# jacobwulffwold/GAN_SR_wind_field

Hardware: AMD Instinct MI355X
Metric: GAN train-steps/sec (G+D fwd+bwd) (higher is better)
Workload: dtype bf16; 1 GPU; C3' full G+D adversarial step: LR 32x32x128 -> HR 128x128x128 (x4), batch 1/GPU, G 16 RRDB nf128 (34.77M), D bf32; preset=C3p, global_batch=1, parallelism=dp1, ranks=1

## Files before the change

### gan_sr_wind_field_amd/_lib.py

```python
from __future__ import annotations

import ctypes as C
import os
from typing import Optional

_HERE = os.path.dirname(os.path.abspath(__file__))
LIB_PATH = os.environ.get("WSR_LIB_PATH") or os.path.join(_HERE, "csrc", "libwindsr_hip.so")

WSR_F32, WSR_BF16 = 0, 1
WSR_EUNSUPPORTED = -2

EXPORTS = [
    "wsr_abi_version", "wsr_error_string", "wsr_reload_env", "wsr_ragan_loss", "wsr_bn_train_stats", "wsr_conv3d_fwd", "wsr_conv3d_dgrad", "wsr_conv3d_wgrad", "wsr_conv3d_wgrad_tri", "wsr_conv3d_wgrad_nparts", "wsr_conv3d_wgrad_parts", "wsr_conv3d_wgrad_parts_x2", "wsr_conv_split_ok", "wsr_unpack_wgrad_reduce_multi", "wsr_conv3d_fwd_tile", "wsr_conv3d_dgrad_tile",
    "wsr_frag_filter_elems", "wsr_pack_filter_frag", "wsr_pack_filter_frag_multi",
    "wsr_pack_filter", "wsr_unpack_wgrad", "wsr_unpack_wgrad_multi", "wsr_lrelu_bwd_inplace", "wsr_chan_axpby", "wsr_chan_sum", "wsr_chan_sum_rows", "wsr_chan_sum_partials", "wsr_upsample2_bwd", "wsr_subpixel_fold", "wsr_subpixel_unfold", "wsr_strided_parity_filters", "wsr_strided_parity_unfold",
    "wsr_planar_to_ndhwc", "wsr_ndhwc_to_planar", "wsr_zfold", "wsr_zunfold", "wsr_wind_gradient", "wsr_wind_gradient_bwd", "wsr_plane_sum", "wsr_linear_rows", "wsr_physics_loss_workspace_floats", "wsr_physics_loss_stats", "wsr_physics_loss_bwd", "wsr_bn_stats", "wsr_bn_mean", "wsr_bn_shard_stats", "wsr_bn_combine_shards", "wsr_bn_finalize", "wsr_bn_apply_lrelu", "wsr_bn_bwd_reduce",
    "wsr_bn_bwd_apply", "wsr_adam_step", "wsr_adam_multi", "wsr_gather_batch",
]


class ConvDesc(C.Structure):

    _fields_ = [(n, C.c_int32) for n in (
        "dtype", "B", "Xi", "Yi", "Zi", "Xo", "Yo", "Zo", "Cin", "in_ctot", "in_off", "Cout", "out_ctot",
        "out_off", "KX", "KY", "KZ", "sx", "sy", "sz", "px", "py", "pz", "upsample_xy", "lat", "lat_ox", "lat_oy",
        "lat_phases", "lat_mz", "lat_oz")]


class Epilogue(C.Structure):

    _fields_ = [
        ("bias", C.c_void_p), ("chan_scale", C.c_void_p), ("res", C.c_void_p),
# ... 78 lines not shown
        "wsr_physics_loss_bwd": [vp, vp, vp, vp, vp, vp, vp, vp, i32, i32, i32, i32, vp],
        "wsr_zunfold": [vp, vp, i32, i32, i32, i32, i64, i32, i32, i32, i32, i32, vp],
        "wsr_bn_stats": [vp, i32, i64, vp, vp, vp, i32, vp],
        "wsr_bn_mean": [vp, vp, f32, vp, i32, vp],
        "wsr_bn_shard_stats": [vp, i32, vp, i32, f32, vp, i32, i32, vp],
        "wsr_bn_combine_shards": [vp, i32, f32, vp, i32, vp, i32, i32, i32, vp],
        "wsr_bn_finalize": [vp, vp, f32, vp, f32, f32, vp, vp, vp, vp, i32, vp],
        "wsr_bn_apply_lrelu": [vp, vp, vp, vp, vp, vp, i32, i64, i32, f32, i32, vp],
        "wsr_bn_bwd_reduce": [vp, vp, vp, vp, vp, i32, i64, i32, f32, vp, vp, i32, vp],
        "wsr_bn_bwd_apply": [vp, vp, vp, vp, vp, vp, vp, f32, vp, f32, i32, i64, i32, vp],
        "wsr_adam_step": [vp, vp, vp, vp, i64, f32, f32, f32, f32, f32, i32, vp],
        "wsr_adam_multi": [vp, i32, C.c_double, C.c_double, C.c_double, C.c_double, C.c_double, i32, vp],
        "wsr_ragan_loss": [vp, vp, vp, vp, vp, vp, i32, vp, vp],
        "wsr_bn_train_stats": [vp, i32, i64, i32, f32, f32, vp, vp, vp, vp, i32, vp],
        "wsr_gather_batch": [vp, i64, vp, i32, i32, i32, i32, i32, i32, i32, vp, vp, vp, vp],
    }
    for name, argtypes in sig.items():
        fn = getattr(L, name)
        fn.argtypes = argtypes
        fn.restype = C.c_int
    L.wsr_frag_filter_elems.argtypes = [i32, i32, i32, i32]
    L.wsr_frag_filter_elems.restype = C.c_int64
    L.wsr_physics_loss_workspace_floats.argtypes = []
    L.wsr_physics_loss_workspace_floats.restype = C.c_int64
    if L.wsr_abi_version() != 9:
        raise RuntimeError("libwindsr_hip.so ABI version mismatch")
    _lib = L
    return L


# ... 5 lines not shown
```

### gan_sr_wind_field_amd/csrc/conv_wgrad.hip

```cpp
#include "common.h"

namespace {

typedef __attribute__((ext_vector_type(4))) short s16x4_t;
typedef s16x4_t __attribute__((address_space(3))) * lds_s16x4_ptr;

struct WgradArgs {
  const char* x;
  const char* dy;
  float* dw;
  int B, Xi, Yi, Zi, Xo, Yo, Zo;
  int Cin, in_ctot, in_off;
  int Cout, out_ctot, out_off;
  int KX, KY, KZ, sx, sy, sz, px, py, pz, ups;
  int M;
  int mchunk;
  int ntiles, ctiles;
  long part_stride;
  int mchunks;
};

template <class T> struct WgCfg;
template <> struct WgCfg<BF16> { static constexpr int KB = 128; };
template <> struct WgCfg<F32> { static constexpr int KB = 64; };
// ... 194 lines not shown

template <class T>
int dispatch_wgrad(WgradArgs& a, hipStream_t st, int* plan, int n_parts) {
  if (a.Cout % 48 == 0 && a.Cin % 48 == 0 && a.Cin % 64 != 0) return launch_wgrad<T, 3, 3>(a, st, plan, n_parts);
  if (a.Cout <= 16)
    return a.Cin <= 16 ? launch_wgrad<T, 1, 1>(a, st, plan, n_parts) : launch_wgrad<T, 1, 4>(a, st, plan, n_parts);
  if (a.Cin <= 16) return launch_wgrad<T, 2, 1>(a, st, plan, n_parts);
  if (a.Cin <= 32) return launch_wgrad<T, 2, 2>(a, st, plan, n_parts);
  return launch_wgrad<T, 2, 4>(a, st, plan, n_parts);
}

}

int wsr_wgrad_tile_bf16(const wsr_conv_t* c, const void* x, const void* dy, float* dw, int tri_base, int tri_step,
                        long part_stride, int n_parts, int* plan, void* stream, const void* x2, int x2_ctot,
                        int x2_c0);

int wsr_wgrad_tile_f32(const wsr_conv_t* c, const void* x, const void* dy, float* dw, long part_stride, int n_parts,
                       int* plan, void* stream, const void* x2, int x2_ctot, int x2_c0);

static int wgrad_any(const wsr_conv_t* c, const void* x, const void* dy, float* dw, int tri_base, int tri_step,
                     long part_stride, int n_parts, int* plan, void* stream, const void* x2 = nullptr, int x2_ctot = 0,
                     int x2_c0 = 0) {
  {
    const int rc = wsr_wgrad_tile_bf16(c, x, dy, dw, tri_base, tri_step, part_stride, n_parts, plan, stream, x2, x2_ctot,
                                       x2_c0);
    if (rc != WSR_EUNSUPPORTED || tri_step > 0) return rc;
  }
  if (c->lat) return WSR_EUNSUPPORTED;
  if (c->dtype == WSR_F32 && tri_step == 0) {
    const int rc = wsr_wgrad_tile_f32(c, x, dy, dw, part_stride, n_parts, plan, stream, x2, x2_ctot, x2_c0);
    if (rc != WSR_EUNSUPPORTED) return rc;
  }
  if (x2) return WSR_EUNSUPPORTED;
  const int epp = c->dtype == WSR_BF16 ? 8 : 4;
  if (c->Cin % epp || c->in_ctot % epp || c->in_off % epp) return WSR_EUNSUPPORTED;
  if (c->out_ctot % epp || c->out_off % epp) return WSR_EUNSUPPORTED;
  if ((long)c->B * c->Xo * c->Yo * c->Zo > 0x7fffffffL) return WSR_EUNSUPPORTED;
  WgradArgs a{};
  a.x = (const char*)x;
  a.dy = (const char*)dy;
// ... 39 lines not shown

extern "C" int wsr_conv3d_wgrad_parts(const wsr_conv_t* c, const void* x, const void* dy, float* parts,
                                      int64_t part_stride, int32_t n_parts, int32_t tri_base, int32_t tri_step,
                                      void* stream) {
  if (!conv_geom_ok(c) || !x || !dy || !parts || tri_base < 0 || tri_step < 0 || n_parts <= 0) return WSR_EINVAL;
  if (part_stride < (int64_t)c->Cout * c->KX * c->KY * c->KZ * c->Cin) return WSR_EINVAL;
  return wgrad_any(c, x, dy, parts, tri_base, tri_step, (long)part_stride, n_parts, nullptr, stream);
}

extern "C" int wsr_conv3d_wgrad_parts_x2(const wsr_conv_t* c, const void* x, const void* x2, int32_t x2_ctot, int32_t x2_c0,
                                         const void* dy, float* parts, int64_t part_stride, int32_t n_parts, void* stream) {
  if (!conv_geom_ok_split(c, x2_c0) || !x || !x2 || !dy || !parts || n_parts <= 0 || x2_ctot <= 0) return WSR_EINVAL;
  if (part_stride < (int64_t)c->Cout * c->KX * c->KY * c->KZ * c->Cin) return WSR_EINVAL;
  return wgrad_any(c, x, dy, parts, 0, 0, (long)part_stride, n_parts, nullptr, stream, x2, x2_ctot, x2_c0);
}
```

### gan_sr_wind_field_amd/csrc/conv_wgrad_tile.hip

```cpp
#include <cstdlib>

#include "common.h"

namespace {

typedef __attribute__((ext_vector_type(4))) short s16x4_t;
typedef s16x4_t __attribute__((address_space(3))) * lds_s16x4_ptr;

struct WgtArgs {
  const unsigned short* x;
  const unsigned short* x2;
  int x2_ctot, x2_c0;
  const unsigned short* dy;
  float* dw;
  const void* zero16;
  int B, Xi, Yi, Zi, Xo, Yo, Zo;
  int Cin, in_ctot, in_off;
  int Cout, out_ctot, out_off;
  int KX, KY, KZ, px, py, pz, ups;
  int TX, TY, TZ;
  int n_chunks, c_chunks, S;
  int tiles_x, tiles_y, tiles_z, ntiles;
  int nbuf;
  int xp_bytes;
// ... 449 lines not shown
  const int taps = a.KX * a.KY * a.KZ;
  if (taps * CT > WAVES * SPW) return WSR_EUNSUPPORTED;
  if (a.x2 && a.x2_c0 % (16 * CT)) return WSR_EUNSUPPORTED;
  {
    static void* zp = nullptr;
    if (!zp) {
      hipError_t e = hipGetSymbolAddress(&zp, HIP_SYMBOL(g_wg_zero16));
      if (e != hipSuccess) return (int)e;
    }
    a.zero16 = zp;
  }
  int tz = a.Zo <= 16 ? a.Zo : ((a.Zo % 16 == 0 || a.Zo > 64) ? 16 : 8);
  if (a.KZ == 1 && a.KX * a.KY > 1 && tz > 4 && a.Zo % 4 == 0 && !WSR_ENV_SET("WSR_CT_NOFLAT")) tz = 4;
  static const int cand[][2] = {{8, 8}, {4, 8}, {4, 4}, {2, 4}, {2, 2}, {1, 2}, {1, 1}};
  int best = -1, best_nbuf = 0;
  const int nbuf_want = taps == 1 ? WSR_ENV_INT("WSR_WG_NBUF", 2) : ((SPW == 4 && CT == 1) ? WSR_ENV_INT("WSR_WG_NBUF_THIN", 2) : 2);
  const int mmax = taps == 1 && nbuf_want > 2 ? WSR_ENV_INT("WSR_WG_MMAX", 64) : 1 << 30;
  for (int nbuf = nbuf_want; nbuf >= 2 && best < 0; --nbuf) {
    for (int ci = 0; ci < 7; ++ci) {
      const int tx = cand[ci][0], ty = cand[ci][1];
      const int M = tx * ty * tz;
      if ((M & 31) || M > mmax) continue;
      if (a.ups && ((tx | ty) & 1)) continue;
      const int L = (tx + a.KX - 1) * (ty + a.KY - 1) * (tz + a.KZ - 1);
      const int xs = CT * round_up(L * 32, 1024), ys = round_up(M * wgt_rby(TN), 1024);
      if (xs / 1024 > wgt_xk(SPW, TN) * WAVES || ys / 1024 > wgt_yk(SPW, TN) * WAVES || L > 65535) continue;
      if (round_up(M * 2, 1024) + nbuf * (xs + ys) > 160 * 1024) continue;
      best = ci;
      best_nbuf = nbuf;
      break;
    }
  }
  if (best < 0) return WSR_EUNSUPPORTED;
  a.TX = cand[best][0]; a.TY = cand[best][1]; a.TZ = tz;
  a.nbuf = best_nbuf;
  const int M = a.TX * a.TY * a.TZ;
  const int L = (a.TX + a.KX - 1) * (a.TY + a.KY - 1) * (a.TZ + a.KZ - 1);
// ... 46 lines not shown
    hipError_t e = hipFuncSetAttribute(reinterpret_cast<const void*>(kern), hipFuncAttributeMaxDynamicSharedMemorySize,
                                       160 * 1024);
    if (e != hipSuccess) return (int)e;
    attr_done[z16] = true;
  }
#ifdef WSR_CT_STAMPS
  a.stamps = getenv("WSR_CT_STAMPS_PTR") ? (unsigned long long*)strtoull(getenv("WSR_CT_STAMPS_PTR"), nullptr, 0) : nullptr;
  a.ablate = WSR_ENV_INT("WSR_CT_ABL", 0);
#endif
  a.prio = WSR_ENV_INT("WSR_CT_PRIO", 0);
  hipLaunchKernelGGL(kern, dim3((unsigned)(combos * a.S)), dim3(WAVES * 64), lds, st, a);
  WSR_LAUNCH_CHECK();
  return 0;
}

}

namespace {
int run_tile(WgtArgs& a, int taps, int Cout, int Cin, hipStream_t st);
}

int wsr_wgrad_tile_bf16(const wsr_conv_t* c, const void* x, const void* dy, float* dw, int tri_base, int tri_step,
                        long part_stride, int n_parts, int* plan, void* stream, const void* x2, int x2_ctot, int x2_c0) {
  if (c->dtype != WSR_BF16 || (c->sx | c->sy | c->sz) != 1) return WSR_EUNSUPPORTED;
  if (x2 && (c->lat || c->upsample_xy || tri_step > 0 || x2_c0 <= 0 || x2_c0 >= c->Cin || x2_c0 % 32 || x2_ctot % 8 ||
             c->Cin - x2_c0 > x2_ctot))
    return WSR_EUNSUPPORTED;
  if (c->lat == 2 && (c->lat_phases || c->lat_mz > 1 || tri_step > 0)) return WSR_EUNSUPPORTED;
  if (c->lat == 3 && (c->lat_phases || tri_step > 0 || c->upsample_xy)) return WSR_EUNSUPPORTED;
  const int taps = c->KX * c->KY * c->KZ;
  if (taps > 128) return WSR_EUNSUPPORTED;
  if (c->Cin % 8 || c->in_ctot % 8 || c->in_off % 8 || c->out_ctot % 8 || c->out_off % 8) return WSR_EUNSUPPORTED;
  if (c->out_off + (c->Cout + 7) / 8 * 8 > c->out_ctot) return WSR_EUNSUPPORTED;
  if (c->KX > 8 || c->KY > 8 || c->KZ > 8) return WSR_EUNSUPPORTED;
  WgtArgs a{};
  a.x = (const unsigned short*)x;
  a.x2 = (const unsigned short*)x2; a.x2_ctot = x2_ctot; a.x2_c0 = x2_c0;
  a.dy = (const unsigned short*)dy;
  a.dw = dw;
  a.B = c->B; a.Xi = c->Xi; a.Yi = c->Yi; a.Zi = c->Zi;
  a.Xo = c->Xo; a.Yo = c->Yo; a.Zo = c->Zo;
  a.Cin = c->Cin; a.in_ctot = c->in_ctot; a.in_off = c->in_off;
  a.Cout = c->Cout; a.out_ctot = c->out_ctot; a.out_off = c->out_off;
  a.KX = c->KX; a.KY = c->KY; a.KZ = c->KZ;
  a.px = c->px; a.py = c->py; a.pz = c->pz;
  a.ups = c->upsample_xy ? 1 : 0;
  a.yl_m = c->lat == 2 ? 2 : 1; a.yl_ox = c->lat == 2 ? c->lat_ox : 0; a.yl_oy = c->lat == 2 ? c->lat_oy : 0;
  a.xl_m = a.xl_mz = 1;
  if (c->lat == 3) {
    a.xl_m = 2; a.xl_ox = c->lat_ox; a.xl_oy = c->lat_oy;
    a.xl_mz = c->lat_mz > 1 ? c->lat_mz : 1; a.xl_oz = c->lat_oz;
  }
  a.tri_base = tri_base; a.tri_step = tri_step;
  a.part_stride = part_stride; a.S_forced = n_parts; a.plan_only = plan ? 1 : 0;
  if (taps == 1 && !c->lat && !c->upsample_xy && c->Zi % 16 != 0 && (c->px | c->py | c->pz) == 0) {
    const long nv = (long)c->Xi * c->Yi * c->Zi;
    if (nv % 128 == 0 && nv / 128 < (1L << 24)) {
      a.Xi = a.Xo = (int)(nv / 128);
      a.Yi = a.Yo = 8;
      a.Zi = a.Zo = 16;
    }
  }
  hipStream_t st = as_stream(stream);
  const int rc = run_tile(a, taps, c->Cout, c->Cin, st);
  if (plan && rc == 0) *plan = a.S;
  return rc;
}

namespace {
int run_tile(WgtArgs& a, int taps, int Cout, int Cin, hipStream_t st) {
  struct { int Cout, Cin; } cc{Cout, Cin};
  auto* c = &cc;
  if (taps == 1) {
    if (c->Cout < 64 || c->Cin < 64) return WSR_EUNSUPPORTED;
    return launch_tile<8, 1, 8>(a, st);
  }
  if (taps > 28) {
    if (c->Cout <= 16) return launch_tile<1, 16, 1>(a, st);
    if (c->Cout % 48 == 0) return launch_tile<3, 16, 1>(a, st);
    return launch_tile<2, 16, 1>(a, st);
  }
  if (taps <= 12 && c->Cout >= 64 && c->Cin >= 64) {
    const int rc = launch_tile<4, 6, 4>(a, st);
    if (rc != WSR_EUNSUPPORTED) return rc;
  }
  const bool small = a.tri_step == 0 && !WSR_ENV_SET("WSR_WG_NOSMALL");
  if (small && taps <= 12 && c->Cout > 16 && c->Cout <= 32) {
    const int rc = launch_tile<2, 3, 2>(a, st);
    if (rc != WSR_EUNSUPPORTED) return rc;
  }
  if (small && c->Cin <= 16 && c->Cout <= 32) {
// ... 13 lines not shown
```

### gan_sr_wind_field_amd/engine.py

```python
from __future__ import annotations

from dataclasses import dataclass
from typing import Callable, Dict, List, Optional, Sequence, Tuple

import torch
from torch import nn

from . import hip_ops as ops
from .hip_ops import ConvGeom

Tensor = torch.Tensor

STACK_DGRAD = __import__("os").environ.get("WSR_STACK_DGRAD", "1") != "0"
STACK_FWD = __import__("os").environ.get("WSR_STACK_FWD", "1") != "0"
FWD_REGROUP = __import__("os").environ.get("WSR_FWD_REGROUP", "0") == "1"
FUSED_BN_STATS = __import__("os").environ.get("WSR_FUSED_BN_STATS", "1") != "0"
GD_INPLACE = __import__("os").environ.get("WSR_GD_INPLACE", "1") != "0"
GD_PINGPONG = __import__("os").environ.get("WSR_GD_PINGPONG", "1") != "0"
ZFOLD = __import__("os").environ.get("WSR_ZFOLD", "1") != "0"
WGRAD_STREAM = int(__import__("os").environ.get("WSR_WGRAD_STREAM", "0"))
F32_TILE = __import__("os").environ.get("WSR_F32_TILE", "1") != "0"
FOLD_D_MASK = __import__("os").environ.get("WSR_FOLD_D_MASK", "0") != "0"
SWAP_THIN_WGRAD = __import__("os").environ.get("WSR_THIN_WGRAD_SWAP", "1") != "0"
SPLIT_CAT = __import__("os").environ.get("WSR_SPLIT_CAT", "1") != "0"
# ... 331 lines not shown
        if DETERMINISTIC:
            dq = d if x2 is None else self._desc(s, B, tuple(x.shape[1:4]), cin_p, 0, g.shape[-1], g_off, cin=cin_p)
            n = self._wgrad_nparts(("w", s.name, B) + tuple(x.shape[1:4]), dq)
            parts = self._arena_take(n * s.cout * s.taps * cin_p, x.device).view(n, s.cout, s.taps, cin_p)
            run = lambda: ops.conv_wgrad_parts(d, x, g, parts, n, x2=x2, x2_c0=x2_c0)
            self._pending_unpack.append((parts[0], out, scale, n, parts[0].numel()))
        else:
            dwp = self._arena_take(s.cout * s.taps * cin_p, x.device)
            run = lambda: ops.conv_wgrad(d, x, g, dwp)
            self._pending_unpack.append((dwp.view(s.cout, s.taps, cin_p), out, scale))
        if self.launch_probe is not None:
            self.launch_probe("wgrad:" + s.name, run)
        else:
            run()

    def wgrad_dense(self, convs: Sequence[ConvSite], buf: Tensor, gd: Tensor, flat: Tensor, space: GradSpace,
                    scratch: Tensor) -> None:
        nf, gc = convs[0].cin, convs[0].cout
        stacked = (self.dt == torch.bfloat16 and len(convs) > 1 and all(
            c.kernel == convs[0].kernel and c.stride == (1, 1, 1) and c.pad == convs[0].pad and c.cout == gc
            and c.cin == nf + i * gc and not c.upsample for i, c in enumerate(convs)))
        if not stacked:
            for i, c in enumerate(convs):
                self.wgrad(c, buf, 0, gd, nf + i * gc, flat, space, scratch)
            return
        B = buf.shape[0]
        cin_w, cout = convs[-1].cin, gc * len(convs)
        g = ConvGeom(cin_w, cout, convs[0].kernel, (1, 1, 1), convs[0].pad)
        d = ops.make_desc(g, self.dt, B, tuple(buf.shape[1:4]), buf.shape[-1], 0, gd.shape[-1], nf)
        taps = convs[0].taps
# ... 129 lines not shown
                run()

    def begin_backward(self, dev) -> None:
        self._pending_unpack = []
        self._arena_off = 0
        self._arena_need = 0
        self._arena_dev = dev
        self._events_used = 0
        if DETERMINISTIC:
            if self._arena is not None and self._arena.device != torch.device(dev):
                self._arena = None
            return
        n = int(self._scratch_elems_total * 1.3) + 4096
        self._arena = torch.zeros(n, dtype=torch.float32, device=dev)

    def _wgrad_nparts(self, key, desc, tri_base: int = 0, tri_step: int = 0) -> int:
        if self._env_gen != ops.ENV_GEN[0]:
            self._nparts.clear()
            self._unpack_tables.clear()
            self._env_gen = ops.ENV_GEN[0]
        n = self._nparts.get(key)
        if n is None:
            n = self._nparts[key] = ops.conv_wgrad_nparts(desc, tri_base, tri_step)
        return n

    def _arena_reserve(self, n_total: int, dev) -> None:
        if not DETERMINISTIC:
            return
        need = n_total + 64 * 64
        bound = max(ARENA_MB << 18, need)
        if self._arena is not None and self._arena.device != torch.device(dev):
            self.flush_unpack()
            self._arena = None
        have = 0 if self._arena is None else self._arena.numel()
        if self._arena_off + need > have and have < bound:
            want = min(bound, max(2 * have, self._arena_off + need, 4 << 18))
            self.flush_unpack()
            self._arena = None
# ... 581 lines not shown
            side = self.side_stream(dev)
            main = torch.cuda.current_stream(dev)
            ring = [gd] + [self._empty(gd.shape, g_out) for _ in range(WGRAD_STREAM - 1)]
            free_ev: List[Optional[torch.cuda.Event]] = [None] * len(ring)
            slot = 0
        if pingpong:
            cur, oth = gd, self._empty(gd.shape, g_out)
            for rdbs, rr_scale in zip(reversed(self.rrdbs), reversed(self.rrdb_scales)):
                nb = len(rdbs)
                for j, (convs, lff, rdb_scale) in enumerate(reversed(rdbs)):
                    bi -= 1
                    buf = bufs[bi]
                    first, lastb = j == 0, j == nb - 1
                    go = cur if first else oth
                    sc = rdb_scale * (rr_scale if first else 1.0)
                    self.wgrad(lff, buf, 0, go, 0, flat, sp, scratch, scale=sc)
                    rows = ops.chan_sum_rows(nf, go.numel() // go.shape[-1])
                    if not rows:
                        raise RuntimeError("LFF bias gradient outside the two-pass sum (set WSR_GD_PINGPONG=0)")
                    pr = self._arena_take(rows * nf, dev).view(rows, nf)
                    ops.chan_sum_partials(go, 0, nf, pr)
                    self._pending_unpack.append((pr[0].view(1, 1, nf), sp.view(flat, lff.bias).view(1, nf, 1), sc, rows, nf))
                    nc = len(convs)
                    last = nf + (nc - 1) * gc
                    self.dgrad(lff, go, 0, oth, 0, (X, Y, nz), alpha=sc, accumulate=nf, acc_src=go if first else None,
                               acc_beta=rr_scale if first else 1.0, res2=cur if lastb else None,
                               mask=(buf, last, last, last + gc) if nc else None)
                    if STACK_DGRAD and self.dense_stackable(convs):
                        self.dgrad_dense(convs, oth, buf, (X, Y, nz))
                    else:
                        for i in reversed(range(nc)):
                            off = nf + i * gc
                            m = (buf, off - gc, off - gc, off) if i > 0 else None
                            self.dgrad(convs[i], oth, off, oth, 0, (X, Y, nz), accumulate=True, mask=m)
                    self.wgrad_dense(convs, buf, oth, flat, sp, scratch)
                    ready(lff.weight, lff.bias, *[c.weight for c in convs])
                cur, oth = oth, cur
# ... 3 lines not shown
                break
            g_skip = g
            if side is not None:
                ops.chan_axpby(ring[slot], 0, g, 0, nf, alpha=rr_scale)
                for convs, lff, rdb_scale in reversed(rdbs):
                    bi -= 1
                    buf = bufs[bi]
                    src, nxt = ring[slot], (slot + 1) % len(ring)
                    dst = ring[nxt]
                    nc = len(convs)
                    last = nf + (nc - 1) * gc
                    ev = self._event()
                    ev.record(main)
                    side.wait_event(ev)
                    with torch.cuda.stream(side):
                        self.wgrad(lff, buf, 0, src, 0, flat, sp, scratch, scale=rdb_scale)
                        rows = ops.chan_sum_rows(nf, src.numel() // src.shape[-1])
                        if not rows:
                            raise RuntimeError("LFF bias gradient outside the two-pass sum (set WSR_WGRAD_STREAM=0)")
                        pr = self._arena_take(rows * nf, dev).view(rows, nf)
                        ops.chan_sum_partials(src, 0, nf, pr)
                        self._pending_unpack.append((pr[0].view(1, 1, nf), sp.view(flat, lff.bias).view(1, nf, 1),
                                                     rdb_scale, rows, nf))
                        fe = self._event()
                        fe.record(side)
                        free_ev[slot] = fe
                    if free_ev[nxt] is not None:
                        main.wait_event(free_ev[nxt])
                        free_ev[nxt] = None
                    self.dgrad(lff, src, 0, dst, 0, (X, Y, nz), alpha=rdb_scale, accumulate=nf, acc_src=src,
                               mask=(buf, last, last, last + gc) if nc else None)
                    if STACK_DGRAD and self.dense_stackable(convs):
                        self.dgrad_dense(convs, dst, buf, (X, Y, nz))
                    else:
                        for i in reversed(range(nc)):
                            off = nf + i * gc
                            m = (buf, off - gc, off - gc, off) if i > 0 else None
                            self.dgrad(convs[i], dst, off, dst, 0, (X, Y, nz), accumulate=True, mask=m)
# ... 4 lines not shown
                        self.wgrad_dense(convs, buf, dst, flat, sp, scratch)
                        ready(lff.weight, lff.bias, *[c.weight for c in convs])
                    slot = nxt
                ops.chan_axpby(g, 0, ring[slot], 0, nf, alpha=1.0, beta=1.0)
                continue
            if inplace:
                go, go_c = gd, nf
                ops.chan_axpby(gd, 0, g, 0, nf, alpha=rr_scale)
            else:
                go, go_c = self._empty(g.shape, g_out), None
                ops.chan_axpby(go, 0, g, 0, nf, alpha=rr_scale)
            for convs, lff, rdb_scale in reversed(rdbs):
                bi -= 1
                buf = bufs[bi]
                tr("rdb_go", bi, go[..., :nf])
                self.wgrad(lff, buf, 0, go, 0, flat, sp, scratch, scale=rdb_scale)
                gb = sp.view(flat, lff.bias)
                rows = ops.chan_sum_rows(nf, go.numel() // go.shape[-1]) if DETERMINISTIC else 0
                if rows:
                    pr = self._arena_take(rows * nf, dev).view(rows, nf)
                    ops.chan_sum_partials(go, 0, nf, pr)
                    self._pending_unpack.append((pr[0].view(1, 1, nf), gb.view(1, nf, 1), rdb_scale, rows, nf))
                elif not ops.chan_sum(go, 0, nf, gb, scale=rdb_scale):
                    gb.copy_(go[..., :nf].float().sum(dim=(0, 1, 2, 3)) * rdb_scale)
                nc = len(convs)
                last = nf + (nc - 1) * gc
                self.dgrad(lff, go, 0, gd, 0, (X, Y, nz), alpha=rdb_scale, accumulate=go_c if inplace else False,
                           mask=(buf, last, last, last + gc) if nc else None)
                if STACK_DGRAD and self.dense_stackable(convs):
                    self.dgrad_dense(convs, gd, buf, (X, Y, nz))
                else:
                    for i in reversed(range(nc)):
                        off = nf + i * gc
                        m = (buf, off - gc, off - gc, off) if i > 0 else None
                        self.dgrad(convs[i], gd, off, gd, 0, (X, Y, nz), accumulate=True, mask=m)
                self.wgrad_dense(convs, buf, gd, flat, sp, scratch)
                if inplace:
                    tr("rdb_gd", bi, gd)
                if not inplace:
# ... 576 lines not shown
```

### gan_sr_wind_field_amd/hip_ops.py

```python
from __future__ import annotations

import ctypes as C
from dataclasses import dataclass
from typing import Optional, Tuple

import torch

from . import _lib
from ._lib import ConvDesc, Epilogue, check

Tensor = torch.Tensor


def dtype_id(dt: torch.dtype) -> int:
    if dt == torch.float32:
        return _lib.WSR_F32
    if dt == torch.bfloat16:
        return _lib.WSR_BF16
    raise TypeError(f"unsupported activation dtype {dt}")


def piece_elems(dt: torch.dtype) -> int:
    return 4 if dt == torch.float32 else 8

# ... 307 lines not shown
    _need_cuda(x, dy, parts)
    if parts.dtype != torch.float32 or not parts.is_contiguous() or parts.shape[0] != n_parts:
        raise ValueError("conv_wgrad_parts wants a contiguous fp32 (n_parts, Cout, taps, Cin) buffer")
    if x2 is not None:
        _need_cuda(x2)
        if tri_step or x2.shape[:-1] != x.shape[:-1] or x2.dtype != x.dtype:
            raise ValueError("x2 must have x's extents and dtype (no stacked form)")
        check(_lib.lib().wsr_conv3d_wgrad_parts_x2(C.byref(desc), _p(x), _p(x2), x2.shape[-1], x2_c0, _p(dy), _p(parts),
                                                   parts[0].numel(), n_parts, _stream()), "conv3d_wgrad_parts_x2")
        return parts
    check(_lib.lib().wsr_conv3d_wgrad_parts(C.byref(desc), _p(x), _p(dy), _p(parts), parts[0].numel(), n_parts, tri_base,
                                            tri_step, _stream()), "conv3d_wgrad_parts")
    return parts


def pack_filter(w: Tensor, dt: torch.dtype, *, transpose: bool = False, kpad: Optional[int] = None,
                out: Optional[Tensor] = None) -> Tensor:
    _need_cuda(w)
    cout, cin = w.shape[:2]
    taps = w[0, 0].numel()
    if not w.is_contiguous() or w.dtype != torch.float32:
        raise ValueError("pack_filter wants a contiguous fp32 (Cout, Cin, KX, KY, KZ) tensor")
    k = cout if transpose else cin
    kpad = pad_channels(k, dt) if kpad is None else kpad
    rows = cin if transpose else cout
    if out is None:
        out = torch.empty((rows, taps, kpad), dtype=dt, device=w.device)
    check(_lib.lib().wsr_pack_filter(_p(w), _p(out), dtype_id(dt), cout, taps, cin, int(transpose), kpad, _stream()),
          "pack_filter")
    return out
# ... 481 lines not shown
```

### include/windsr_hip.h

```cpp
#ifndef WINDSR_HIP_H
#define WINDSR_HIP_H

#include <stdint.h>

#ifdef __cplusplus
extern "C" {
#endif

#define WSR_ABI_VERSION 9

enum wsr_dtype { WSR_F32 = 0, WSR_BF16 = 1 };

enum wsr_error {
  WSR_OK = 0,
  WSR_EINVAL = -1,
  WSR_EUNSUPPORTED = -2
};

typedef struct wsr_conv {
  int32_t dtype;
  int32_t B;
  int32_t Xi, Yi, Zi;
  int32_t Xo, Yo, Zo;
  int32_t Cin, in_ctot, in_off;
// ... 66 lines not shown
                         int32_t transpose, int32_t dtype, void* stream);
typedef struct wsr_pack_job {
  const float* w;
  void* out;
  int32_t Cout, Cin, KX, KY, KZ, transpose;
  int32_t c_lo, c_n, red_off, red_total, row_off, rows_total;
} wsr_pack_job_t;
int wsr_pack_filter_frag_multi(const wsr_pack_job_t* jobs_dev, int32_t n_jobs, int32_t dtype, void* stream);

int wsr_conv3d_wgrad(const wsr_conv_t* c, const void* x, const void* dy, float* dw, void* stream);
int wsr_conv3d_wgrad_nparts(const wsr_conv_t* c, int32_t tri_base, int32_t tri_step, int32_t* n_parts);
int wsr_conv3d_wgrad_parts(const wsr_conv_t* c, const void* x, const void* dy, float* parts, int64_t part_stride,
                           int32_t n_parts, int32_t tri_base, int32_t tri_step, void* stream);
int wsr_conv3d_wgrad_parts_x2(const wsr_conv_t* c, const void* x, const void* x2, int32_t x2_ctot, int32_t x2_c0,
                              const void* dy, float* parts, int64_t part_stride, int32_t n_parts, void* stream);
int wsr_conv3d_wgrad_tri(const wsr_conv_t* c, const void* x, const void* dy, float* dw, int32_t tri_base,
                         int32_t tri_step, void* stream);

int wsr_pack_filter(const float* w, void* out, int32_t dtype, int32_t Cout, int32_t taps,
                    int32_t Cin, int32_t transpose, int32_t kpad, void* stream);
int wsr_unpack_wgrad(const float* src, float* dst, int32_t Cout, int32_t taps, int32_t Cin,
                     int32_t kpad, float scale, int32_t accumulate, void* stream);

typedef struct wsr_unpack_job {
  const float* src;
  float* dst;
  int32_t Cout, taps, Cin, kpad;
  float scale;
  int32_t accumulate;
  int32_t n_parts;
// ... 97 lines not shown
```

Before: 11.32 train-steps/s.

## Add dedicated 1x1x1 wgrad kernel with fused bias-gradient reduction for LFF convs

Replaces the generic tiled wgrad path for 1x1x1 convolutions with a new kernel that streams voxel chunks into LDS through a three-stage DMA pipeline and computes dW with MFMA. The same kernel also accumulates the bias gradient by multiplying dy against a ones fragment, so the separate channel-sum partials pass over the gradient is dropped for the RRDB local-feature-fusion convs. The engine gains a wgrad_bias helper that uses the fused deterministic parts path when it is available and otherwise falls back to the old route. The old taps==1 reshaping hack and the NBUF/MMAX env knobs are removed. The cost is extra MFMA work on the waves that handle the bias and a larger LDS footprint.

```diff
diff --git a/gan_sr_wind_field_amd/_lib.py b/gan_sr_wind_field_amd/_lib.py
--- a/gan_sr_wind_field_amd/_lib.py
+++ b/gan_sr_wind_field_amd/_lib.py
@@ -15,7 +15,8 @@
     "wsr_frag_filter_elems", "wsr_pack_filter_frag", "wsr_pack_filter_frag_multi",
     "wsr_pack_filter", "wsr_unpack_wgrad", "wsr_unpack_wgrad_multi", "wsr_lrelu_bwd_inplace", "wsr_chan_axpby", "wsr_chan_sum", "wsr_chan_sum_rows", "wsr_chan_sum_partials", "wsr_upsample2_bwd", "wsr_subpixel_fold", "wsr_subpixel_unfold", "wsr_strided_parity_filters", "wsr_strided_parity_unfold",
     "wsr_planar_to_ndhwc", "wsr_ndhwc_to_planar", "wsr_zfold", "wsr_zunfold", "wsr_wind_gradient", "wsr_wind_gradient_bwd", "wsr_plane_sum", "wsr_linear_rows", "wsr_physics_loss_workspace_floats", "wsr_physics_loss_stats", "wsr_physics_loss_bwd", "wsr_bn_stats", "wsr_bn_mean", "wsr_bn_shard_stats", "wsr_bn_combine_shards", "wsr_bn_finalize", "wsr_bn_apply_lrelu", "wsr_bn_bwd_reduce",
-    "wsr_bn_bwd_apply", "wsr_adam_step", "wsr_adam_multi", "wsr_gather_batch",
+    "wsr_bn_bwd_apply", "wsr_adam_step", "wsr_adam_multi", "wsr_gather_batch", "wsr_conv3d_wgrad_bias_nparts",
+    "wsr_conv3d_wgrad_parts_bias",
 ]
 
 
@@ -124,6 +125,8 @@
         "wsr_ragan_loss": [vp, vp, vp, vp, vp, vp, i32, vp, vp],
         "wsr_bn_train_stats": [vp, i32, i64, i32, f32, f32, vp, vp, vp, vp, i32, vp],
         "wsr_gather_batch": [vp, i64, vp, i32, i32, i32, i32, i32, i32, i32, vp, vp, vp, vp],
+        "wsr_conv3d_wgrad_bias_nparts": [C.POINTER(ConvDesc), C.POINTER(C.c_int32)],
+        "wsr_conv3d_wgrad_parts_bias": [C.POINTER(ConvDesc), vp, vp, vp, i64, i32, vp, vp],
     }
     for name, argtypes in sig.items():
         fn = getattr(L, name)
diff --git a/gan_sr_wind_field_amd/csrc/conv_wgrad.hip b/gan_sr_wind_field_amd/csrc/conv_wgrad.hip
--- a/gan_sr_wind_field_amd/csrc/conv_wgrad.hip
+++ b/gan_sr_wind_field_amd/csrc/conv_wgrad.hip
@@ -232,7 +232,7 @@
 
 int wsr_wgrad_tile_bf16(const wsr_conv_t* c, const void* x, const void* dy, float* dw, int tri_base, int tri_step,
                         long part_stride, int n_parts, int* plan, void* stream, const void* x2, int x2_ctot,
-                        int x2_c0);
+                        int x2_c0, float* bias);
 
 int wsr_wgrad_tile_f32(const wsr_conv_t* c, const void* x, const void* dy, float* dw, long part_stride, int n_parts,
                        int* plan, void* stream, const void* x2, int x2_ctot, int x2_c0);
@@ -242,7 +242,7 @@
                      int x2_c0 = 0) {
   {
     const int rc = wsr_wgrad_tile_bf16(c, x, dy, dw, tri_base, tri_step, part_stride, n_parts, plan, stream, x2, x2_ctot,
-                                       x2_c0);
+                                       x2_c0, nullptr);
     if (rc != WSR_EUNSUPPORTED || tri_step > 0) return rc;
   }
   if (c->lat) return WSR_EUNSUPPORTED;
@@ -312,3 +312,20 @@
   if (part_stride < (int64_t)c->Cout * c->KX * c->KY * c->KZ * c->Cin) return WSR_EINVAL;
   return wgrad_any(c, x, dy, parts, 0, 0, (long)part_stride, n_parts, nullptr, stream, x2, x2_ctot, x2_c0);
 }
+
+extern "C" int wsr_conv3d_wgrad_bias_nparts(const wsr_conv_t* c, int32_t* n_parts) {
+  if (!conv_geom_ok(c) || !n_parts) return WSR_EINVAL;
+  int plan = 0;
+  static float placeholder[4];
+  const int rc = wsr_wgrad_tile_bf16(c, nullptr, nullptr, nullptr, 0, 0, 1, 0, &plan, nullptr, nullptr, 0, 0, placeholder);
+  *n_parts = plan;
+  return rc;
+}
+
+extern "C" int wsr_conv3d_wgrad_parts_bias(const wsr_conv_t* c, const void* x, const void* dy, float* parts,
+                                           int64_t part_stride, int32_t n_parts, float* bias_parts, void* stream) {
+  if (!conv_geom_ok(c) || !x || !dy || !parts || !bias_parts || n_parts <= 0) return WSR_EINVAL;
+  if (part_stride < (int64_t)c->Cout * c->KX * c->KY * c->KZ * c->Cin) return WSR_EINVAL;
+  return wsr_wgrad_tile_bf16(c, x, dy, parts, 0, 0, (long)part_stride, n_parts, nullptr, stream, nullptr, 0, 0,
+                             bias_parts);
+}
diff --git a/gan_sr_wind_field_amd/csrc/conv_wgrad_tile.hip b/gan_sr_wind_field_amd/csrc/conv_wgrad_tile.hip
--- a/gan_sr_wind_field_amd/csrc/conv_wgrad_tile.hip
+++ b/gan_sr_wind_field_amd/csrc/conv_wgrad_tile.hip
@@ -487,13 +487,12 @@
   if (a.KZ == 1 && a.KX * a.KY > 1 && tz > 4 && a.Zo % 4 == 0 && !WSR_ENV_SET("WSR_CT_NOFLAT")) tz = 4;
   static const int cand[][2] = {{8, 8}, {4, 8}, {4, 4}, {2, 4}, {2, 2}, {1, 2}, {1, 1}};
   int best = -1, best_nbuf = 0;
-  const int nbuf_want = taps == 1 ? WSR_ENV_INT("WSR_WG_NBUF", 2) : ((SPW == 4 && CT == 1) ? WSR_ENV_INT("WSR_WG_NBUF_THIN", 2) : 2);
-  const int mmax = taps == 1 && nbuf_want > 2 ? WSR_ENV_INT("WSR_WG_MMAX", 64) : 1 << 30;
+  const int nbuf_want = (SPW == 4 && CT == 1) ? WSR_ENV_INT("WSR_WG_NBUF_THIN", 2) : 2;
   for (int nbuf = nbuf_want; nbuf >= 2 && best < 0; --nbuf) {
     for (int ci = 0; ci < 7; ++ci) {
       const int tx = cand[ci][0], ty = cand[ci][1];
       const int M = tx * ty * tz;
-      if ((M & 31) || M > mmax) continue;
+      if (M & 31) continue;
       if (a.ups && ((tx | ty) & 1)) continue;
       const int L = (tx + a.KX - 1) * (ty + a.KY - 1) * (tz + a.KZ - 1);
       const int xs = CT * round_up(L * 32, 1024), ys = round_up(M * wgt_rby(TN), 1024);
@@ -570,6 +569,210 @@
   return 0;
 }
 
+constexpr int LF_WAVES = 16, LF_NT = LF_WAVES * 64;
+constexpr int LF_MV = 128;
+constexpr int LF_CT = 4;
+constexpr int LF_YB = LF_MV * 256;
+constexpr int LF_XP = LF_MV * 32;
+constexpr int LF_BUF = LF_YB + LF_CT * LF_XP;
+constexpr int LF_NBUF = 3;
+constexpr int LF_RS = 68;
+static_assert(LF_YB / 1024 + LF_CT * LF_XP / 1024 == 3 * LF_WAVES, "three 1 KB DMA units per wave and stage");
+static_assert((4 * 128 * LF_RS + 4 * 128) * 4 <= LF_NBUF * LF_BUF, "the K-group reduce fits the stage buffers");
+
+struct LffArgs {
+  const unsigned short* x;
+  const unsigned short* x2;
+  int x2_ctot, x2_c0;
+  const unsigned short* dy;
+  float* dw;
+  float* bias;
+  const void* zero16;
+  long V;
+  int Cin, in_ctot, in_off, Cout, out_ctot, out_off;
+  int c_groups, n_chunks, S, nstages;
+  long part_stride;
+};
+
+__global__ __launch_bounds__(LF_NT) void wgrad_lff_kernel(const LffArgs a) {
+  extern __shared__ __attribute__((aligned(16))) char smem[];
+  const int t = threadIdx.x, lane = t & 63;
+  const int wave = __builtin_amdgcn_readfirstlane(t >> 6);
+  typedef __attribute__((address_space(3))) char* lptr_t;
+  const unsigned lds0 = (unsigned)(unsigned long)(lptr_t)smem;
+
+  int bid = xcd_remap(blockIdx.x, gridDim.x);
+  const int cg = bid % a.c_groups;
+  bid /= a.c_groups;
+  const int nc = bid % a.n_chunks;
+  const int s0 = bid / a.n_chunks;
+  const int c0 = cg * 16 * LF_CT, n0 = nc * 128;
+  const bool second = a.x2 != nullptr && c0 >= a.x2_c0;
+  const unsigned short* xt = second ? a.x2 : a.x;
+  const int x_ctot = second ? a.x2_ctot : a.in_ctot;
+  const int x_off = second ? c0 - a.x2_c0 : a.in_off + c0;
+
+  int yv[2], yrel[2];
+  bool yok[2];
+#pragma unroll
+  for (int k = 0; k < 2; ++k) {
+    const int u = wave + LF_WAVES * k;
+    const int v = 4 * u + (lane >> 4), sl = lane & 15;
+    const int oct = 2 * ((sl >> 1) ^ (v & 7)) + (sl & 1);
+    yv[k] = v;
+    yok[k] = n0 + 8 * oct < a.Cout;
+    yrel[k] = v * a.out_ctot + n0 + 8 * oct;
+  }
+  const int xv = (wave & 3) * 32 + (lane >> 1);
+  const int xch = 16 * (wave >> 2) + 8 * (lane & 1);
+  const bool xok = c0 + xch < a.Cin;
+  const int xrel = xv * x_ctot + xch;
+
+  const unsigned short* zsrc = reinterpret_cast<const unsigned short*>(a.zero16);
+  auto issue = [&](int stage, int buf) {
+    const long vox0 = (long)stage * LF_MV;
+    const bool inner = vox0 + LF_MV <= a.V;
+    const unsigned dst = lds0 + buf * LF_BUF;
+    const unsigned short* yb = a.dy + vox0 * a.out_ctot + a.out_off;
+#pragma unroll
+    for (int k = 0; k < 2; ++k) {
+      const bool ok = yok[k] && (inner || vox0 + yv[k] < a.V);
+      glds16(ok ? yb + yrel[k] : zsrc, __builtin_amdgcn_readfirstlane(dst + (wave + LF_WAVES * k) * 1024));
+    }
+    const unsigned short* xb = xt + vox0 * x_ctot + x_off;
+    const bool ok = xok && (inner || vox0 + xv < a.V);
+    glds16(ok ? xb + xrel : zsrc, __builtin_amdgcn_readfirstlane(dst + LF_YB + wave * 1024));
+  };
+
+  const int ks = wave >> 2, nh = (wave >> 1) & 1, cp = wave & 1;
+  const bool do_bias = a.bias != nullptr && cg == 0 && cp == 0;
+  const int G = lane >> 4, q = (lane & 15) >> 2, p = lane & 3;
+  const int m_lo = ks * 32 + 16 * (G >> 1) + 4 * (G & 1) + q;
+  const int sw = m_lo & 7;
+  f32x4_t acc[4][2], accb[4];
+#pragma unroll
+  for (int i = 0; i < 4; ++i) {
+    accb[i] = f32x4_t{0.f, 0.f, 0.f, 0.f};
+#pragma unroll
+    for (int j = 0; j < 2; ++j) acc[i][j] = f32x4_t{0.f, 0.f, 0.f, 0.f};
+  }
+  const uint4 ones = make_uint4(0x3F803F80u, 0x3F803F80u, 0x3F803F80u, 0x3F803F80u);
+
+  const int ntl = (a.nstages - s0 + a.S - 1) / a.S;
+  constexpr int DT = LF_NBUF - 1, UPT = 3;
+  int bi = 0, bc = 0;
+  for (int it = 0;; ++it) {
+    if (it < ntl) issue(s0 + it * a.S, bi);
+    bi = bi + 1 == LF_NBUF ? 0 : bi + 1;
+    if (it >= DT) {
+      const char* Ys = smem + bc * LF_BUF;
+      const char* Xs = Ys + LF_YB;
+      bc = bc + 1 == LF_NBUF ? 0 : bc + 1;
+      const char* ylo = Ys + m_lo * 256 + p * 8;
+      const char* xlo = Xs + m_lo * 32 + p * 8 + 2 * cp * LF_XP;
+      uint4 af[4], bf[2];
+#pragma unroll
+      for (int i = 0; i < 4; ++i) {
+        const char* lo = ylo + (((4 * nh + i) ^ sw) << 5);
+        af[i] = tr_frag(lo, lo + 8 * 256);
+      }
+#pragma unroll
+      for (int j = 0; j < 2; ++j) bf[j] = tr_frag(xlo + j * LF_XP, xlo + j * LF_XP + 8 * 32);
+#pragma unroll
+      for (int i = 0; i < 4; ++i)
+#pragma unroll
+        for (int j = 0; j < 2; ++j)
+          acc[i][j] = __builtin_amdgcn_mfma_f32_16x16x32_bf16(__builtin_bit_cast(bf16x8_t, af[i]),
+                                                              __builtin_bit_cast(bf16x8_t, bf[j]), acc[i][j], 0, 0, 0);
+      if (do_bias) {
+#pragma unroll
+        for (int i = 0; i < 4; ++i)
+          accb[i] = __builtin_amdgcn_mfma_f32_16x16x32_bf16(__builtin_bit_cast(bf16x8_t, af[i]),
+                                                            __builtin_bit_cast(bf16x8_t, ones), accb[i], 0, 0, 0);
+      }
+    }
+    const int tnext = it - DT + 1;
+    if (tnext >= 0) {
+      int later = ntl - 1 - tnext;
+      later = later < 0 ? 0 : (later > it - tnext ? it - tnext : later);
+      dma_wait_upto(later * UPT);
+    }
+    __syncthreads();
+    if (tnext >= ntl) break;
+  }
+
+  float* red = reinterpret_cast<float*>(smem);
+  float* redb = red + 4 * 128 * LF_RS;
+#pragma unroll
+  for (int i = 0; i < 4; ++i)
+#pragma unroll
+    for (int j = 0; j < 2; ++j)
+#pragma unroll
+      for (int r = 0; r < 4; ++r)
+        red[(ks * 128 + 16 * (4 * nh + i) + 4 * G + r) * LF_RS + 16 * (2 * cp + j) + (lane & 15)] = acc[i][j][r];
+  if (do_bias && (lane & 15) == 0) {
+#pragma unroll
+    for (int i = 0; i < 4; ++i)
+#pragma unroll
+      for (int r = 0; r < 4; ++r) redb[ks * 128 + 16 * (4 * nh + i) + 4 * G + r] = accb[i][r];
+  }
+  __syncthreads();
+  float* const dwp = a.dw + (long)s0 * a.part_stride;
+  const bool store = a.part_stride > 0;
+#pragma unroll
+  for (int e = 0; e < 128 * 16 * LF_CT / LF_NT; ++e) {
+    const int idx = t + LF_NT * e;
+    const int nl = idx >> 6, cl = idx & 63;
+    const int n = n0 + nl, c = c0 + cl;
+    const float* s = red + nl * LF_RS + cl;
+    const float v = ((s[0] + s[128 * LF_RS]) + s[2 * 128 * LF_RS]) + s[3 * 128 * LF_RS];
+    if (n < a.Cout && c < a.Cin) {
+      float* d = dwp + (long)n * a.Cin + c;
+      if (store) *d = v;
+      else atomicAdd(d, v);
+    }
+  }
+  if (a.bias != nullptr && cg == 0 && t < 128 && n0 + t < a.Cout)
+    a.bias[(long)s0 * a.Cout + n0 + t] = ((redb[t] + redb[128 + t]) + redb[256 + t]) + redb[384 + t];
+}
+
+int launch_lff(LffArgs& a, bool plan_only, int S_forced, hipStream_t st) {
+  if (a.Cout < 64 || a.Cin < 64) return WSR_EUNSUPPORTED;
+  if (a.x2 && a.x2_c0 % (16 * LF_CT)) return WSR_EUNSUPPORTED;
+  if (a.bias && a.part_stride <= 0) return WSR_EUNSUPPORTED;
+  const long nst = (a.V + LF_MV - 1) / LF_MV;
+  if (nst > 0x7fffffffL || a.V * (long)(a.in_ctot > a.out_ctot ? a.in_ctot : a.out_ctot) > 0x7fffffffffffL)
+    return WSR_EUNSUPPORTED;
+  a.nstages = (int)nst;
+  a.c_groups = (a.Cin + 16 * LF_CT - 1) / (16 * LF_CT);
+  a.n_chunks = (a.Cout + 127) / 128;
+  int S = 256 / (a.c_groups * a.n_chunks);
+  if (S < 1) S = 1;
+  if (S > a.nstages) S = a.nstages;
+  a.S = S;
+  if (plan_only) return 0;
+  if (a.part_stride > 0 && S_forced != a.S) return WSR_EINVAL;
+  {
+    static void* zp = nullptr;
+    if (!zp) {
+      hipError_t e = hipGetSymbolAddress(&zp, HIP_SYMBOL(g_wg_zero16));
+      if (e != hipSuccess) return (int)e;
+    }
+    a.zero16 = zp;
+  }
+  constexpr size_t lds = (size_t)LF_NBUF * LF_BUF;
+  static bool attr_done = false;
+  if (!attr_done) {
+    hipError_t e = hipFuncSetAttribute(reinterpret_cast<const void*>(wgrad_lff_kernel),
+                                       hipFuncAttributeMaxDynamicSharedMemorySize, (int)lds);
+    if (e != hipSuccess) return (int)e;
+    attr_done = true;
+  }
+  hipLaunchKernelGGL(wgrad_lff_kernel, dim3((unsigned)(a.S * a.c_groups * a.n_chunks)), dim3(LF_NT), lds, st, a);
+  WSR_LAUNCH_CHECK();
+  return 0;
+}
+
 }
 
 namespace {
@@ -577,7 +780,8 @@
 }
 
 int wsr_wgrad_tile_bf16(const wsr_conv_t* c, const void* x, const void* dy, float* dw, int tri_base, int tri_step,
-                        long part_stride, int n_parts, int* plan, void* stream, const void* x2, int x2_ctot, int x2_c0) {
+                        long part_stride, int n_parts, int* plan, void* stream, const void* x2, int x2_ctot, int x2_c0,
+                        float* bias) {
   if (c->dtype != WSR_BF16 || (c->sx | c->sy | c->sz) != 1) return WSR_EUNSUPPORTED;
   if (x2 && (c->lat || c->upsample_xy || tri_step > 0 || x2_c0 <= 0 || x2_c0 >= c->Cin || x2_c0 % 32 || x2_ctot % 8 ||
              c->Cin - x2_c0 > x2_ctot))
@@ -589,6 +793,23 @@
   if (c->Cin % 8 || c->in_ctot % 8 || c->in_off % 8 || c->out_ctot % 8 || c->out_off % 8) return WSR_EUNSUPPORTED;
   if (c->out_off + (c->Cout + 7) / 8 * 8 > c->out_ctot) return WSR_EUNSUPPORTED;
   if (c->KX > 8 || c->KY > 8 || c->KZ > 8) return WSR_EUNSUPPORTED;
+  if (taps == 1) {
+    if (c->lat || c->upsample_xy || tri_step > 0 || (c->px | c->py | c->pz) != 0) return WSR_EUNSUPPORTED;
+    LffArgs l{};
+    l.x = (const unsigned short*)x;
+    l.x2 = (const unsigned short*)x2; l.x2_ctot = x2_ctot; l.x2_c0 = x2_c0;
+    l.dy = (const unsigned short*)dy;
+    l.dw = dw;
+    l.bias = bias;
+    l.V = (long)c->B * c->Xo * c->Yo * c->Zo;
+    l.Cin = c->Cin; l.in_ctot = c->in_ctot; l.in_off = c->in_off;
+    l.Cout = c->Cout; l.out_ctot = c->out_ctot; l.out_off = c->out_off;
+    l.part_stride = part_stride;
+    const int rc = launch_lff(l, plan != nullptr, n_parts, as_stream(stream));
+    if (plan && rc == 0) *plan = l.S;
+    return rc;
+  }
+  if (bias) return WSR_EUNSUPPORTED;
   WgtArgs a{};
   a.x = (const unsigned short*)x;
   a.x2 = (const unsigned short*)x2; a.x2_ctot = x2_ctot; a.x2_c0 = x2_c0;
@@ -609,14 +830,6 @@
   }
   a.tri_base = tri_base; a.tri_step = tri_step;
   a.part_stride = part_stride; a.S_forced = n_parts; a.plan_only = plan ? 1 : 0;
-  if (taps == 1 && !c->lat && !c->upsample_xy && c->Zi % 16 != 0 && (c->px | c->py | c->pz) == 0) {
-    const long nv = (long)c->Xi * c->Yi * c->Zi;
-    if (nv % 128 == 0 && nv / 128 < (1L << 24)) {
-      a.Xi = a.Xo = (int)(nv / 128);
-      a.Yi = a.Yo = 8;
-      a.Zi = a.Zo = 16;
-    }
-  }
   hipStream_t st = as_stream(stream);
   const int rc = run_tile(a, taps, c->Cout, c->Cin, st);
   if (plan && rc == 0) *plan = a.S;
@@ -627,10 +840,6 @@
 int run_tile(WgtArgs& a, int taps, int Cout, int Cin, hipStream_t st) {
   struct { int Cout, Cin; } cc{Cout, Cin};
   auto* c = &cc;
-  if (taps == 1) {
-    if (c->Cout < 64 || c->Cin < 64) return WSR_EUNSUPPORTED;
-    return launch_tile<8, 1, 8>(a, st);
-  }
   if (taps > 28) {
     if (c->Cout <= 16) return launch_tile<1, 16, 1>(a, st);
     if (c->Cout % 48 == 0) return launch_tile<3, 16, 1>(a, st);
diff --git a/gan_sr_wind_field_amd/engine.py b/gan_sr_wind_field_amd/engine.py
--- a/gan_sr_wind_field_amd/engine.py
+++ b/gan_sr_wind_field_amd/engine.py
@@ -369,6 +369,37 @@
         else:
             run()
 
+    def wgrad_bias(self, s: ConvSite, x: Tensor, g: Tensor, flat: Tensor, space: GradSpace, scratch: Tensor,
+                   scale: float) -> None:
+        dev = x.device
+        gb = space.view(flat, s.bias)
+        B = x.shape[0]
+        cin_p = self.cp(s.cin)
+        d = self._desc(s, B, tuple(x.shape[1:4]), x.shape[-1], 0, g.shape[-1], 0, cin=cin_p)
+        n = self._wgrad_nparts(("wb", s.name, B) + tuple(x.shape[1:4]), d, bias=True) if DETERMINISTIC else 0
+        if n:
+            self._arena_reserve((n * s.cout * cin_p + 63) // 64 * 64 + (n * s.cout + 63) // 64 * 64, dev)
+            parts = self._arena_take(n * s.cout * cin_p, dev).view(n, s.cout, 1, cin_p)
+            bp = self._arena_take(n * s.cout, dev).view(n, s.cout)
+            self._pending_unpack.append((parts[0], space.view(flat, s.weight), scale, n, parts[0].numel()))
+            self._pending_unpack.append((bp[0].view(1, 1, s.cout), gb.view(1, s.cout, 1), scale, n, s.cout))
+            run = lambda: ops.conv_wgrad_parts_bias(d, x, g, parts, n, bp)
+            if self.launch_probe is not None:
+                self.launch_probe("wgrad:" + s.name, run)
+            else:
+                run()
+            return
+        self.wgrad(s, x, 0, g, 0, flat, space, scratch, scale=scale)
+        rows = ops.chan_sum_rows(s.cout, g.numel() // g.shape[-1]) if DETERMINISTIC else 0
+        if rows:
+            pr = self._arena_take(rows * s.cout, dev).view(rows, s.cout)
+            ops.chan_sum_partials(g, 0, s.cout, pr)
+            self._pending_unpack.append((pr[0].view(1, 1, s.cout), gb.view(1, s.cout, 1), scale, rows, s.cout))
+        elif DETERMINISTIC:
+            raise RuntimeError("bias gradient outside the two-pass channel sum")
+        elif not ops.chan_sum(g, 0, s.cout, gb, scale=scale):
+            gb.copy_(g[..., :s.cout].float().sum(dim=(0, 1, 2, 3)) * scale)
+
     def wgrad_dense(self, convs: Sequence[ConvSite], buf: Tensor, gd: Tensor, flat: Tensor, space: GradSpace,
                     scratch: Tensor) -> None:
         nf, gc = convs[0].cin, convs[0].cout
@@ -528,14 +559,15 @@
         n = int(self._scratch_elems_total * 1.3) + 4096
         self._arena = torch.zeros(n, dtype=torch.float32, device=dev)
 
-    def _wgrad_nparts(self, key, desc, tri_base: int = 0, tri_step: int = 0) -> int:
+    def _wgrad_nparts(self, key, desc, tri_base: int = 0, tri_step: int = 0, bias: bool = False) -> int:
         if self._env_gen != ops.ENV_GEN[0]:
             self._nparts.clear()
             self._unpack_tables.clear()
             self._env_gen = ops.ENV_GEN[0]
         n = self._nparts.get(key)
         if n is None:
-            n = self._nparts[key] = ops.conv_wgrad_nparts(desc, tri_base, tri_step)
+            n = self._nparts[key] = (ops.conv_wgrad_bias_nparts(desc) if bias
+                                     else ops.conv_wgrad_nparts(desc, tri_base, tri_step))
         return n
 
     def _arena_reserve(self, n_total: int, dev) -> None:
@@ -1147,13 +1179,7 @@
                     first, lastb = j == 0, j == nb - 1
                     go = cur if first else oth
                     sc = rdb_scale * (rr_scale if first else 1.0)
-                    self.wgrad(lff, buf, 0, go, 0, flat, sp, scratch, scale=sc)
-                    rows = ops.chan_sum_rows(nf, go.numel() // go.shape[-1])
-                    if not rows:
-                        raise RuntimeError("LFF bias gradient outside the two-pass sum (set WSR_GD_PINGPONG=0)")
-                    pr = self._arena_take(rows * nf, dev).view(rows, nf)
-                    ops.chan_sum_partials(go, 0, nf, pr)
-                    self._pending_unpack.append((pr[0].view(1, 1, nf), sp.view(flat, lff.bias).view(1, nf, 1), sc, rows, nf))
+                    self.wgrad_bias(lff, buf, go, flat, sp, scratch, sc)
                     nc = len(convs)
                     last = nf + (nc - 1) * gc
                     self.dgrad(lff, go, 0, oth, 0, (X, Y, nz), alpha=sc, accumulate=nf, acc_src=go if first else None,
@@ -1187,14 +1213,7 @@
                     ev.record(main)
                     side.wait_event(ev)
                     with torch.cuda.stream(side):
-                        self.wgrad(lff, buf, 0, src, 0, flat, sp, scratch, scale=rdb_scale)
-                        rows = ops.chan_sum_rows(nf, src.numel() // src.shape[-1])
-                        if not rows:
-                            raise RuntimeError("LFF bias gradient outside the two-pass sum (set WSR_WGRAD_STREAM=0)")
-                        pr = self._arena_take(rows * nf, dev).view(rows, nf)
-                        ops.chan_sum_partials(src, 0, nf, pr)
-                        self._pending_unpack.append((pr[0].view(1, 1, nf), sp.view(flat, lff.bias).view(1, nf, 1),
-                                                     rdb_scale, rows, nf))
+                        self.wgrad_bias(lff, buf, src, flat, sp, scratch, rdb_scale)
                         fe = self._event()
                         fe.record(side)
                         free_ev[slot] = fe
@@ -1229,15 +1248,7 @@
                 bi -= 1
                 buf = bufs[bi]
                 tr("rdb_go", bi, go[..., :nf])
-                self.wgrad(lff, buf, 0, go, 0, flat, sp, scratch, scale=rdb_scale)
-                gb = sp.view(flat, lff.bias)
-                rows = ops.chan_sum_rows(nf, go.numel() // go.shape[-1]) if DETERMINISTIC else 0
-                if rows:
-                    pr = self._arena_take(rows * nf, dev).view(rows, nf)
-                    ops.chan_sum_partials(go, 0, nf, pr)
-                    self._pending_unpack.append((pr[0].view(1, 1, nf), gb.view(1, nf, 1), rdb_scale, rows, nf))
-                elif not ops.chan_sum(go, 0, nf, gb, scale=rdb_scale):
-                    gb.copy_(go[..., :nf].float().sum(dim=(0, 1, 2, 3)) * rdb_scale)
+                self.wgrad_bias(lff, buf, go, flat, sp, scratch, rdb_scale)
                 nc = len(convs)
                 last = nf + (nc - 1) * gc
                 self.dgrad(lff, go, 0, gd, 0, (X, Y, nz), alpha=rdb_scale, accumulate=go_c if inplace else False,
diff --git a/gan_sr_wind_field_amd/hip_ops.py b/gan_sr_wind_field_amd/hip_ops.py
--- a/gan_sr_wind_field_amd/hip_ops.py
+++ b/gan_sr_wind_field_amd/hip_ops.py
@@ -345,6 +345,26 @@
     return parts
 
 
+def conv_wgrad_bias_nparts(desc: ConvDesc) -> int:
+    n = C.c_int32(0)
+    rc = _lib.lib().wsr_conv3d_wgrad_bias_nparts(C.byref(desc), C.byref(n))
+    if rc == _lib.WSR_EUNSUPPORTED:
+        return 0
+    check(rc, "conv3d_wgrad_bias_nparts")
+    return int(n.value)
+
+
+def conv_wgrad_parts_bias(desc: ConvDesc, x: Tensor, dy: Tensor, parts: Tensor, n_parts: int, bias_parts: Tensor) -> Tensor:
+    _need_cuda(x, dy, parts, bias_parts)
+    if parts.dtype != torch.float32 or not parts.is_contiguous() or parts.shape[0] != n_parts:
+        raise ValueError("conv_wgrad_parts_bias wants a contiguous fp32 (n_parts, Cout, 1, Cin) buffer")
+    if bias_parts.dtype != torch.float32 or not bias_parts.is_contiguous() or bias_parts.shape != (n_parts, desc.Cout):
+        raise ValueError("conv_wgrad_parts_bias wants a contiguous fp32 (n_parts, Cout) bias buffer")
+    check(_lib.lib().wsr_conv3d_wgrad_parts_bias(C.byref(desc), _p(x), _p(dy), _p(parts), parts[0].numel(), n_parts,
+                                                 _p(bias_parts), _stream()), "conv3d_wgrad_parts_bias")
+    return parts
+
+
 def pack_filter(w: Tensor, dt: torch.dtype, *, transpose: bool = False, kpad: Optional[int] = None,
                 out: Optional[Tensor] = None) -> Tensor:
     _need_cuda(w)
diff --git a/include/windsr_hip.h b/include/windsr_hip.h
--- a/include/windsr_hip.h
+++ b/include/windsr_hip.h
@@ -104,6 +104,9 @@
                            int32_t n_parts, int32_t tri_base, int32_t tri_step, void* stream);
 int wsr_conv3d_wgrad_parts_x2(const wsr_conv_t* c, const void* x, const void* x2, int32_t x2_ctot, int32_t x2_c0,
                               const void* dy, float* parts, int64_t part_stride, int32_t n_parts, void* stream);
+int wsr_conv3d_wgrad_bias_nparts(const wsr_conv_t* c, int32_t* n_parts);
+int wsr_conv3d_wgrad_parts_bias(const wsr_conv_t* c, const void* x, const void* dy, float* parts, int64_t part_stride,
+                                int32_t n_parts, float* bias_parts, void* stream);
 int wsr_conv3d_wgrad_tri(const wsr_conv_t* c, const void* x, const void* dy, float* dw, int32_t tri_base,
                          int32_t tri_step, void* stream);
 
```

New measurement: 11.45 train-steps/s (median of 6 runs). +1.2%, better.
